# joey156/MECH5845M-WBC-for-Legged-Manipulator

Measured on AMD Instinct MI355X. Metric: wbc_qp_solves_per_sec, higher is better.
Workload: dtype f64

## Files before the change

### mech5845m-wbc-for-legged-manipulator_amd/csrc/wbc_api.hip

```cpp
#include <hip/hip_runtime.h>
#include <stdarg.h>
#include <stdio.h>
#include <string.h>
#include <new>
#include <vector>
#include "wbc_device.h"

using namespace wbc;

static thread_local char g_err[512] = "";
static int fail(int code, const char* fmt, ...) {
  va_list ap;
  va_start(ap, fmt);
  vsnprintf(g_err, sizeof g_err, fmt, ap);
  va_end(ap);
  return code;
}
#define HIP_TRY(expr)                                                                       \
  do {                                                                                      \
    hipError_t e_ = (expr);                                                                 \
    if (e_ != hipSuccess) return fail(WBC_E_HIP, "%s: %s", #expr, hipGetErrorString(e_));   \
  } while (0)

enum TickPath : int { TICK_GENERAL = 0, TICK_SIM3 = 1, TICK_SIM3P = 2, TICK_ORTHP = 3, TICK_BOXP = 4 };
// ... 28 lines not shown
  int packed_min_batch;
  int packed_kernel;
  int posture_par, last_posture_par;
  int packed_box;
  int packed_orth;
  int refine;
  int warm_start;
  int32_t* d_defer;
  unsigned long long* d_dstat;
  int wave_order;
  WaveOrder* d_worder;
  int worder_reset;
  int worder_B;
  uint32_t tick_seq;
  int packed_update, last_update_packed;
  int last_orth;
  int last_qp_path;
  int last_path;
  int max_nj, max_nf;
  int rot;
  unsigned long long* d_prof;
  double *d_pu, *d_pq;
  void* d_roll;
};

static bool is_identity(const double* R) {
  static const double I[9] = {1, 0, 0, 0, 1, 0, 0, 0, 1};
  for (int i = 0; i < 9; ++i)
    if (R[i] != I[i]) return false;
  return true;
// ... 83 lines not shown

extern "C" void wbc_model_destroy(WbcModel* m) { delete m; }

extern "C" void wbc_batch_destroy(WbcBatch* b);
extern "C" int wbc_batch_create(const WbcModel* const* models, int n_models, int max_batch, int device_id, WbcBatch** out) {
  if (!out || n_models < 0 || n_models > WBC_MAX_MODELS || (n_models > 0 && !models) || max_batch < 1)
    return fail(WBC_E_ARG, "wbc_batch_create: bad arguments (n_models %d, max_batch %d)", n_models, max_batch);
  int ndev = 0;
  if (hipGetDeviceCount(&ndev) != hipSuccess || ndev < 1)
    return fail(WBC_E_HIP, "wbc_batch_create: no HIP device visible (this library has no CPU fallback)");
  if (device_id < 0 || device_id >= ndev) return fail(WBC_E_ARG, "wbc_batch_create: device %d of %d", device_id, ndev);
  HIP_TRY(hipSetDevice(device_id));
  WbcBatch* b = new (std::nothrow) WbcBatch;
  if (!b) return fail(WBC_E_ARG, "out of memory");
  memset(b, 0, sizeof *b);
  b->device_id = device_id; b->n_models = n_models; b->max_batch = max_batch; b->presolve = 1; b->presolve_orth = 1; b->packed_update = 1; b->sim3_kernel = 1; b->sing_tol = 1e-7; b->wave_order = 1;
  b->jtj_mfma = -1; b->refine = 1; b->packed_min_batch = WBC_SIM3P_MIN_BATCH; b->warm_start = 0; b->packed_kernel = 1; b->packed_orth = 1; b->packed_box = 1; b->posture_par = 1;
  std::vector<DevModel> dm(n_models);
  for (int i = 0; i < n_models; ++i) {
    if (!models[i]) { delete b; return fail(WBC_E_ARG, "wbc_batch_create: model %d is null", i); }
    b->models[i] = models[i];
    dm[i] = models[i]->dev;
    if (models[i]->blob.njoints > b->max_nj) b->max_nj = models[i]->blob.njoints;
    if (models[i]->blob.nframes > b->max_nf) b->max_nf = models[i]->blob.nframes;
    if (models[i]->dev.rot_mask) b->rot = 1;
  }
#define HIP_TRY_B(expr)                                                                                              \
  do {                                                                                                               \
    hipError_t e_ = (expr);                                                                                          \
    if (e_ != hipSuccess) { wbc_batch_destroy(b); return fail(WBC_E_HIP, "%s: %s", #expr, hipGetErrorString(e_)); }  \
  } while (0)
// ... 100 lines not shown
    if (jp < 0) return;
    if (jp != joint_id && ((M.col_subtree[M.idx_v_of[jp]] >> joint_id) & 1u)) return;
    zero |= 1u << i;
    if (literal) pert |= 1u << qi;
  }
  if (mode == WBC_JOINT_MANI) return;
  P->post_static = 1; P->post_zero = zero; P->post_pert = pert;
  uint32_t dofs = 0;
  for (int k = 0; k < M.nv; ++k) if ((pert >> M.col_q[k]) & 1u) dofs |= 1u << k;
  bool dep = c.con_com != 0 && dofs != 0;
  if (c.con_trunk && (M.frame_support[WBC_FR_TRUNK] & dofs)) dep = true;
  for (int e = 0; e < WBC_NEE; ++e) if (c.con_ee[e] && (M.frame_support[WBC_FR_EE0 + e] & dofs)) dep = true;
  P->post_fk2 = dep ? 1 : 0;
}

static bool build_pk_fk(const DevModel& M, int need_depth, DevPlan* P) {
  for (int i = 0; i < 32; ++i) P->pk_scq[i] = -1;
  for (int L = 0; L < 5; ++L) {
    int cnt = 0;
    for (int i = 0; i < 16; ++i) { memset(&P->pk_fk[L][i], 0, sizeof P->pk_fk[L][i]); P->pk_fk[L][i].joint = -1; }
    for (int j = 2; j < M.njoints; ++j)
      if (M.depth[j] == L + 2 && M.depth[j] <= need_depth) {
        if (cnt < 16) {
          DevPlan::PkJoint& r = P->pk_fk[L][cnt];
          const bool rev = M.jtype[j] >= WBC_JT_RX && M.jtype[j] <= WBC_JT_RZ;
          r.joint = j; r.parent = M.parent[j]; r.a0 = 3 * M.ax0[j]; r.a1 = 3 * M.ax1[j]; r.a2 = 3 * M.ax2[j];
          r.rev = rev ? 1 : 0; r.q_idx = M.idx_q[j]; r.t0 = M.tp[j][0]; r.t1 = M.tp[j][1]; r.t2 = M.tp[j][2]; r.rot = (M.rot_mask >> j) & 1u;
          if (rev && j < 32) P->pk_scq[j] = M.idx_q[j];
        }
        ++cnt;
      }
    if (cnt > 16) return false;
  }
  return true;
}

static bool build_q_tables(const DevModel& M, DevPlan* P, bool need_subtree) {
  if (M.njoints > 22 || M.maxdepth > 7) return false;
  for (int i = 0; i < 32; ++i) { P->q_scq[i] = -1; memset(&P->q_dof[i], 0, sizeof P->q_dof[i]); P->q_dof[i].bl = P->q_dof[i].red = -1; memset(&P->q_jm[i], 0, sizeof P->q_jm[i]); }
  for (int L = 0; L < 6; ++L) {
    int cnt = 0;
    for (int i = 0; i < 16; ++i) { memset(&P->q_fk[L][i], 0, sizeof P->q_fk[L][i]); P->q_fk[L][i].joint = -1; }
    for (int j = 2; j < M.njoints; ++j)
      if (M.depth[j] == L + 2) {
        if (cnt >= 16) return false;
        DevPlan::PkJoint& r = P->q_fk[L][cnt++];
        const bool rev = M.jtype[j] >= WBC_JT_RX && M.jtype[j] <= WBC_JT_RZ;
        r.joint = j; r.parent = M.parent[j]; r.a0 = 3 * M.ax0[j]; r.a1 = 3 * M.ax1[j]; r.a2 = 3 * M.ax2[j];
// ... 232 lines not shown
  b->configured[mi] = true;
  b->plan_host[mi] = DevPlan();
  b->mrows = m; b->prows = p; b->mcart = mcart;
  HIP_TRY(hipMemcpy(b->d_cfgs + mi, cfg, sizeof *cfg, hipMemcpyHostToDevice));
  DevPlan plan;
  build_plan(b->models[mi]->dev, *cfg, p, &plan);
  b->plan_host[mi] = plan;
  HIP_TRY(hipMemcpy(b->d_plans + mi, &plan, sizeof plan, hipMemcpyHostToDevice));
  b->worder_reset = 1;
  return WBC_OK;
}

extern "C" int wbc_task_rows(const WbcBatch* b) { return b ? b->mrows : WBC_E_ARG; }
extern "C" int wbc_constraint_rows(const WbcBatch* b) { return b ? b->prows : WBC_E_ARG; }

extern "C" int wbc_batch_set_option(WbcBatch* b, const char* name, int value) {
  if (!b || !name) return fail(WBC_E_ARG, "wbc_batch_set_option: null");
  if (!strcmp(name, "jtj_mfma")) { b->jtj_mfma = value < 0 ? -1 : (value ? 1 : 0); return WBC_OK; }
  if (!strcmp(name, "presolve")) { b->presolve = value; return WBC_OK; }
  if (!strcmp(name, "presolve_orth")) { b->presolve_orth = value; return WBC_OK; }
  if (!strcmp(name, "orth_qr")) { b->orth_qr = value; return WBC_OK; }
  if (!strcmp(name, "packed_update")) { b->packed_update = value; return WBC_OK; }
  if (!strcmp(name, "presolve_tol_exp")) { double t = 1.0; for (int i = 0; i < value; ++i) t *= 0.1; b->sing_tol = t; return WBC_OK; }
  if (!strcmp(name, "sim3_kernel")) { b->sim3_kernel = value; return WBC_OK; }
  if (!strcmp(name, "packed_kernel")) { b->packed_kernel = value; return WBC_OK; }
  if (!strcmp(name, "wave_order")) { b->wave_order = value < 0 ? 0 : (value > 2 ? 2 : value); return WBC_OK; }
  if (!strcmp(name, "packed_min_batch")) { b->packed_min_batch = value < 1 ? 1 : value; return WBC_OK; }
  if (!strcmp(name, "packed_orth")) { b->packed_orth = value; return WBC_OK; }
  if (!strcmp(name, "packed_box")) { b->packed_box = value; return WBC_OK; }
  if (!strcmp(name, "posture_par")) { b->posture_par = value; return WBC_OK; }
  if (!strcmp(name, "dbg_alias_inputs")) { b->dbg_alias = value; return WBC_OK; }
  if (!strcmp(name, "warm_start")) { b->warm_start = value != 0; return WBC_OK; }
  if (!strcmp(name, "refine")) { b->refine = value > 0; return WBC_OK; }
  if (!strcmp(name, "count_pivoted")) { b->count_pivoted = value != 0; return WBC_OK; }
  if (!strcmp(name, "dbg_force_defer")) { b->force_defer = value != 0; return WBC_OK; }
  if (!strcmp(name, "dbg_stop")) {
#ifdef WBC_ABLATE
    b->dbg_stop = value; return WBC_OK;
#else
    return value == 0 ? WBC_OK : fail(WBC_E_UNSUPPORTED, "dbg_stop needs the ablation build of the library (make -C csrc ablate; WBC_HIP_LIB=.../libwbc_hip_ablate.so)");
#endif
  }
  if (!strcmp(name, "grid")) { if (value < 1) return fail(WBC_E_ARG, "grid must be >= 1"); b->grid = value; return WBC_OK; }
  return fail(WBC_E_ARG, "unknown option %s", name);
}

extern "C" int wbc_batch_get_stat(WbcBatch* b, const char* name, void* stream, int64_t* out) {
  if (!b || !name || !out) return fail(WBC_E_ARG, "wbc_batch_get_stat: null");
  HIP_TRY(hipSetDevice(b->device_id));
  if (!strcmp(name, "last_path")) { *out = b->last_path; return WBC_OK; }
  if (!strcmp(name, "last_qp_path")) { *out = b->last_qp_path; return WBC_OK; }
  if (!strcmp(name, "last_update_packed")) { *out = b->last_update_packed; return WBC_OK; }
  if (!strcmp(name, "last_posture_par")) { *out = b->last_posture_par; return WBC_OK; }
  if (!strcmp(name, "last_orth")) { *out = (b->last_path == TICK_GENERAL || b->last_path == TICK_ORTHP) ? b->last_orth : 0; return WBC_OK; }
  if (!strcmp(name, "deferred_last")) {
    *out = 0;
    if (b->last_path >= TICK_SIM3P) {
      if (!b->d_dstat) return WBC_OK;
      unsigned long long v = 0;
      HIP_TRY(hipStreamSynchronize((hipStream_t)stream));
      HIP_TRY(hipMemcpy(&v, b->d_dstat, sizeof v, hipMemcpyDeviceToHost));
      *out = ((uint32_t)(v >> 32) == b->tick_seq) ? (int64_t)(v & 0xFFFFFFFFull) : 0;
      return WBC_OK;
    }
    if (!b->d_defer || b->last_path == TICK_GENERAL) return WBC_OK;
    int32_t c = 0;
    HIP_TRY(hipStreamSynchronize((hipStream_t)stream));
// ... 153 lines not shown
    }
    if (all_static && !a.in.q_con) { a.post_static = 1; return WBC_OK; }
  }
  if (!b->d_pu) {
    HIP_TRY(hipMalloc((void**)&b->d_pu, sizeof(double) * WBC_V_STRIDE * (size_t)b->max_batch));
    HIP_TRY(hipMalloc((void**)&b->d_pq, sizeof(double) * WBC_Q_STRIDE * (size_t)b->max_batch));
  }
  if (int rc = run_posture(b, B, a.in.q, a.in.model_id, b->d_pu, b->d_pq, stream)) return rc;
  a.in.posture_u = b->d_pu;
  if (literal && !a.in.q_con) a.in.q_con = b->d_pq;
  return WBC_OK;
}

static void fill_args(KernelArgs& a, const WbcBatch* b, int B, double dt) {
  memset(&a, 0, sizeof a);
  a.models = b->d_models; a.cfgs = b->d_cfgs; a.plans = b->d_plans; a.n_models = b->n_models; a.rot = b->rot;
  a.B = B; a.mrows = b->mrows; a.prows = b->prows; a.mcart = b->mcart; a.jtj_mfma = b->jtj_mfma < 0 ? (b->mcart >= WBC_MFMA_AUTO_ROWS) : b->jtj_mfma; a.presolve = b->presolve; a.presolve_orth = b->presolve_orth ? 1 + any_orth_plan(b) : 0; a.orth_qr = b->orth_qr; a.refine = b->refine; a.sing_tol = b->sing_tol; a.dbg_alias = b->dbg_alias; a.dt = dt;
  a.prof = b->d_prof; a.dbg_stop = b->dbg_stop;
  a.fk_nj = b->max_nj; a.fk_nf = b->max_nf;
}

static int launch_rc(int e, const char* what) {
  if (e == WBC_E_UNSUPPORTED) return fail(e, "%s kernel: no variant of it is built for this combination of inputs", what);
  return e ? fail(WBC_E_HIP, "%s kernel launch failed: %s", what, hipGetErrorString((hipError_t)e)) : WBC_OK;
}
static int launch_update_auto(WbcBatch* b, UpdateArgs& u, int B, void* stream) {
  bool packed = b->packed_update != 0;
  for (int i = 0; i < b->n_models && packed; ++i) packed = b->configured[i] && b->plan_host[i].pk_update_ok != 0;
  u.plans = b->d_plans;
  b->last_update_packed = packed;
  return packed ? launch_update_packed(u, stream) : launch_update(u, B, stream);
}
static bool packed_eligible(const WbcBatch* b, const KernelArgs& a) {
  const bool qcon = a.in.q_con || a.in.posture_u;
  bool packed = b->packed_kernel && a.B >= b->packed_min_batch &&
                !b->count_pivoted && !(b->dbg_stop > 0 && b->dbg_stop < 100) && !b->dbg_alias;
  for (int i = 0; i < b->n_models && packed; ++i) packed = qcon ? (b->plan_host[i].packed_ok_pu != 0) : (b->plan_host[i].packed_ok != 0);
  return packed;
}
static bool sim3_eligible(const WbcBatch* b, const KernelArgs& a) {
  if (!b->sim3_kernel || !b->presolve || b->n_models < 1) return false;
  if (b->jtj_mfma > 0) return false;
  if (a.in.com_target || a.in.com_target_vel) return false;
  if (b->prows > WBC_SIM3_MAXP || b->mcart > 12) return false;
// ... 66 lines not shown
        }
      }
      if (b->d_worder && b->worder_reset) {
        HIP_TRY(hipMemsetAsync(b->d_worder, 0, WO_NS * sizeof(WaveOrder), (hipStream_t)stream));
        b->worder_reset = 0;
      }
      a.worder = b->d_worder;
    }
    b->worder_B = a.worder ? a.B : 0;
  }
  return WBC_OK;
}
static int launch_tick_auto(WbcBatch* b, KernelArgs& a, int B, void* stream, const WbcTaskParams* tp = nullptr) {
  const TickPath path = select_tick_path(b, a, tp);
  b->last_path = path;
  if (path == TICK_GENERAL) b->last_orth = a.presolve && a.presolve_orth == 2 && !(a.ws_in || a.ws_out);
  else if (path >= TICK_ORTHP) b->last_orth = path == TICK_ORTHP;
  int rc = prepare_tick(b, a, stream, path);
  if (rc) return rc;
  switch (path) {
    case TICK_GENERAL: return launch_rc(launch_tick(a, MODE_TICK, grid_tick(b, B), stream, tp), "tick");
    case TICK_SIM3P: return launch_rc(launch_tick_sim3p(a, stream, tp), "packed sim3 tick");
    case TICK_ORTHP: return launch_rc(launch_tick_orthp(a, stream, b->plan_host[0].q_ok == 2, tp), "packed orth tick");
    case TICK_BOXP: return launch_rc(launch_tick_boxp(a, stream, tp), "packed box tick");
    case TICK_SIM3: break;
  }
  if ((rc = launch_rc(launch_tick_sim3(a, B, stream), "sim3 tick"))) return rc;
  if ((rc = launch_rc(launch_tick_deferred(a, stream), "deferred tick")))
    (void)hipMemsetAsync(b->d_defer, 0, sizeof(int32_t), (hipStream_t)stream);
  return rc;
// ... 291 lines not shown
```

### mech5845m-wbc-for-legged-manipulator_amd/csrc/wbc_device.h

```cpp
#pragma once
#include <stddef.h>
#include <stdint.h>
#include "../../include/wbc.h"

namespace wbc {

constexpr int NV = WBC_V_STRIDE;
constexpr int NQ = WBC_Q_STRIDE;
constexpr int NL = 32;

struct DevModel {
  int32_t nq, nv, njoints, maxdepth, nframes, pad_[3];
  int32_t parent[NL], depth[NL], jtype[NL], idx_q[NL];
  int32_t ax0[NL], ax1[NL], ax2[NL];
  double tp[NL][3];
  double mass[NL], com[NL][3];
  int32_t col_joint[NL], col_lin[NL], col_ang[NL], col_q[NL];
  uint32_t col_subtree[NL];
  int32_t idx_v_of[NL];
  int32_t frame_joint[WBC_MAX_FRAMES];
  double frame_p[WBC_MAX_FRAMES][3];
  uint32_t frame_support[WBC_MAX_FRAMES];
  double total_mass;
  uint32_t rot_mask, pad1_;
// ... 38 lines not shown
  uint32_t post_pert;
  int32_t mp_ok, mp_n, mp_pad_[2];
  int32_t mp_i[32], mp_qi[32], mp_joint[32];
  int32_t mp_chain[32][8];
  uint32_t mp_prev[32];
  uint32_t mp_all;
  uint32_t mp_prevmode;
  uint32_t flags;
  uint32_t task_ee_mask, con_ee_mask;
  int32_t rowstart[4];
  int32_t legd[12];
  int32_t Fd[WBC_PLAN_NR];
  uint32_t redsup[WBC_MAX_FRAMES];
  int32_t pos[32];
  int32_t lidx[32];
};

enum Mode : int { MODE_TICK = 0, MODE_ASSEMBLE = 1, MODE_FK = 2 };

constexpr int WO_NCLS = 6;
constexpr int WO_SW = 127;
constexpr int WO_CAP = 4 * WO_SW;
constexpr int WO_NS = 256;
struct WaveOrder {
  unsigned long long word[2];
  uint32_t cur;
  uint32_t B;
  uint32_t off[8];
  uint32_t pad_[18];
};
static_assert(sizeof(WaveOrder) == 128, "one slice block per 128-byte line");
inline size_t wave_order_bytes(int max_batch) {
  const int ns = ((max_batch + 3) / 4 + WO_SW - 1) / WO_SW;
  return ns > WO_NS ? 0 : WO_NS * sizeof(WaveOrder) + sizeof(uint32_t) * 2 * WO_NS * WO_NCLS * (size_t)WO_CAP;
}

struct KernelArgs {
  const DevModel* models;
  const WbcConfig* cfgs;
  const DevPlan* plans;
  int32_t B, mrows, prows, mcart;
  int32_t n_models, pad0_;
  int32_t post_static;
  int32_t dbg_alias;
  int32_t dbg_stop;
  int32_t jtj_mfma, presolve;
  int32_t fk_nj, fk_nf;
  int32_t* defer;
  int32_t* pivot_count;
  int32_t* defer_aux;
  int32_t dbg_force_defer;
  int32_t packed_trunk;
  uint32_t tick_seq;
  unsigned long long* defer_stat;
  int32_t presolve_orth;
  int32_t orth_qr;
  int32_t refine;
// ... 48 lines not shown
  const DevModel* models;
  const WbcConfig* cfgs;
  const DevPlan* plans;
  int32_t B, n_models;
  const double* q;
  const int32_t* model_id;
  double *u, *q_after;
  int32_t rot;
};

struct UpdateArgs {
  const DevModel* models;
  const WbcConfig* cfgs;
  const DevPlan* plans;
  int32_t B, n_models;
  int32_t mode, pad_;
  const double *q_cur, *q_next, *imu, *foot_targets;
  const int32_t* model_id;
  double* q_new;
  double *ee_target, *prev_ee_target, *trunk_target, *prev_trunk_target, *ee_prev_rot, *trunk_prev_rot;
  const double *ee_ref_rot, *trunk_ref_euler, *ee_step, *trunk_step;
  double* grip_trace;
  const int32_t *status, *iters;
  int32_t *status_max, *iters_sum;
  int32_t rot;
};

int launch_tick(const KernelArgs& a, int mode, int grid, void* stream, const WbcTaskParams* tp = nullptr);
int launch_tick_sim3(const KernelArgs& a, int grid, void* stream);
int launch_tick_sim3p(const KernelArgs& a, void* stream, const WbcTaskParams* tp = nullptr);
int launch_tick_boxp(const KernelArgs& a, void* stream, const WbcTaskParams* tp = nullptr);
// ... 17 lines not shown
```

### mech5845m-wbc-for-legged-manipulator_amd/csrc/wbc_k_misc.hip

```cpp
#include "wbc_packed.h"

namespace wbc {

template <int NM, bool WARM = false>
__global__ void __launch_bounds__(64, 2) wbc_qp_kernel(const QpArgs A) {
  __shared__ Smem S;
  S.cl[threadIdx.x] = 0.0;
#pragma unroll 1
  for (int b = blockIdx.x; b < A.B; b += gridDim.x) {
    int lane = threadIdx.x, n = A.n, p = A.p, m = A.m;
    asm volatile("" : "+v"(lane), "+s"(n), "+s"(p), "+s"(m));
    const int li = li_clamp(lane);
    double g = 0.0;
    if (m > 0) {
      const double* Ab = A.A + (size_t)b * m * n;
      const double* bb = A.bvec + (size_t)b * m;
      if (A.use_mfma) {
        jtj_mfma(S, lane, m, [&](int r, int c) -> double {
          if (r >= m) return 0.0;
          if (c < n) return Ab[(size_t)r * n + c];
          return (c == NV) ? bb[r] : 0.0;
        });
        g = (lane < n) ? -S.npv[li] : 0.0;
        if (n < NV) {
// ... 722 lines not shown
  const double eet = (A.ee_target && s < 15) ? A.ee_target[b * 15 + s] : 0.0;
  const double ees = (A.ee_target && A.ee_step && s < 15) ? A.ee_step[b * 15 + s] : 0.0;
  double rref[3] = {0.0, 0.0, 0.0};
  if (A.ee_prev_rot && A.ee_ref_rot) {
#pragma unroll
    for (int h = 0; h < 3; ++h) if (16 * h + s < 45) rref[h] = A.ee_ref_rot[b * 45 + 16 * h + s];
  }
  const double tt = (A.trunk_target && s < 3) ? A.trunk_target[b * 3 + s] : 0.0;
  const double tts = (A.trunk_target && A.trunk_step && s < 3) ? A.trunk_step[b * 3 + s] : 0.0;
  const double ter = (A.trunk_prev_rot && A.trunk_ref_euler && s < 3) ? A.trunk_ref_euler[b * 3 + s] : 0.0;
  int st = 0, stm = 0, it = 0, its = 0;
  if (s == 0) {
    if (A.status_max) { st = A.status[b]; stm = A.status_max[b]; }
    if (A.iters_sum) { it = A.iters[b]; its = A.iters_sum[b]; }
  }
  DevPlan::PkJoint fkn = P.pk_fk[0][s];
  const int scq0 = P.pk_scq[(2 + s) & 31], scq1 = P.pk_scq[(18 + s) & 31];
  const int fr = (s < 4) ? WBC_FR_EE0 + s : ((s == 4) ? WBC_FR_TRUNK : WBC_FR_EE0 + 4);
  const int fjoint = M.frame_joint[fr];
  const double f0 = M.frame_p[fr][0], f1 = M.frame_p[fr][1], f2 = M.frame_p[fr][2];
  const int tjoint = M.frame_joint[WBC_FR_TRUNK];
  U.q[s] = c0; U.q[16 + s] = c1;
  if (s < 12) U.ft[s] = ft;
  WSYNC();
  const double* const qv = U.q;
  double* const oMi = U.oMi;
  if (scq0 >= 0) { const SinCos t = sincos_cw(qv[scq0]); U.sc[2 * (2 + s)] = t.s; U.sc[2 * (2 + s) + 1] = t.c; }
  if (scq1 >= 0) { const SinCos t = sincos_cw(qv[scq1]); U.sc[2 * (18 + s)] = t.s; U.sc[2 * (18 + s) + 1] = t.c; }
  if (s == 0) {
    double Rt[9];
    quat_to_R(qv + 3, Rt);
#pragma unroll
    for (int c = 0; c < 3; ++c)
#pragma unroll
      for (int rr = 0; rr < 3; ++rr) oMi[12 + 3 * c + rr] = Rt[3 * rr + c];
    oMi[12 + 9] = qv[0]; oMi[12 + 10] = qv[1]; oMi[12 + 11] = qv[2];
  }
  WSYNC();
#pragma unroll 1
  for (int L = 0; L < 5; ++L) {
    const DevPlan::PkJoint fk = fkn;
    if (L + 1 < 5) fkn = P.pk_fk[L + 1][s];
    const int j = fk.joint;
    if (j >= 0) {
      const bool rev = fk.rev != 0;
      const int a0 = fk.a0, a1 = fk.a1, a2 = fk.a2;
      const double* Pp = oMi + 12 * fk.parent;
      const double sn = rev ? U.sc[2 * j] : 0.0, cs = rev ? U.sc[2 * j + 1] : 1.0;
      const double pris = rev ? 0.0 : qv[fk.q_idx];
      if (ROT && fk.rot) {
        fk_place_rot_lds(oMi + 12 * j, Pp, M.rp[j], a0, a1, a2, sn, cs, pris);
      } else {
        double Av[3], Bv[3], Cv[3], Pv[3];
#pragma unroll
        for (int rr = 0; rr < 3; ++rr) { Av[rr] = Pp[a0 + rr]; Bv[rr] = Pp[a1 + rr]; Cv[rr] = Pp[a2 + rr]; Pv[rr] = Pp[9 + rr]; }
        double* Po = oMi + 12 * j;
#pragma unroll
        for (int rr = 0; rr < 3; ++rr) {
          Po[a0 + rr] = Av[rr];
          Po[a1 + rr] = cs * Bv[rr] + sn * Cv[rr];
          Po[a2 + rr] = cs * Cv[rr] - sn * Bv[rr];
          Po[9 + rr] = Pv[rr] + Av[rr] * (fk.t0 + pris) + Bv[rr] * fk.t1 + Cv[rr] * fk.t2;
        }
      }
    }
    WSYNC();
  }
  if (s < 6) {
    const double* Pj = oMi + 12 * fjoint;
#pragma unroll
    for (int rr = 0; rr < 3; ++rr) U.pf[4 * s + rr] = Pj[9 + rr] + Pj[rr] * f0 + Pj[3 + rr] * f1 + Pj[6 + rr] * f2;
  }
  WSYNC();
  const double* Pt = oMi + 12 * tjoint;
  double WPA[3], BPA[3], base[3];
#pragma unroll
  for (int i = 0; i < 3; ++i) {
    const double t = U.pf[4 * 4 + i];
    WPA[i] = (U.ft[i] + U.ft[3 + i] + U.ft[6 + i] + U.ft[9 + i]) / 4;
    BPA[i] = ((U.pf[i] - t) + (U.pf[4 + i] - t) + (U.pf[8 + i] - t) + (U.pf[12 + i] - t)) / 4;
  }
// ... 86 lines not shown
```

### mech5845m-wbc-for-legged-manipulator_amd/csrc/wbc_k_sim3p.hip

```cpp
#include "wbc_packed.h"

namespace wbc {

#ifdef WBC_ABLATE
#define PSTOP(k, val) do { if (A.dbg_stop == 100 + (k)) { if (valid) { A.out.qdot[(size_t)b * NV + s] = (val); if (s == 0) A.out.status[b] = 0; } return; } } while (0)
#else
#define PSTOP(k, val) do { } while (0)
#endif
#ifndef SIM3P_WAVES
#define SIM3P_WAVES 2
#endif
template <bool WARM, bool TRUNK = false, bool QCON = false, bool ROT = false, bool TP = false>
#ifdef SIM3P_NUM_VGPR
__attribute__((amdgpu_waves_per_eu(SIM3P_NUM_VGPR, SIM3P_NUM_VGPR)))
#endif
__global__ void __launch_bounds__(64, SIM3P_WAVES) wbc_tick_sim3p_kernel(const KernelArgs A, const DevModel* __restrict__ models,
                                                               const WbcConfig* __restrict__ cfgs, const DevPlan* __restrict__ plans,
                                                               const WbcTaskParams* __restrict__ tps) {
#ifdef SIM3P_NUM_VGPR
  extern __shared__ double dyn_lds_[];
  union SUU { SmemP P; Smem G; };
  SUU& SU = *reinterpret_cast<SUU*>(dyn_lds_);
#else
  __shared__ union { SmemP P; Smem G; } SU;
// ... 124 lines not shown
      for (int k = 0; k < 6; ++k) {
        const double2a t0 = lds2(At2 + k * 6), t1 = lds2(At2 + k * 6 + 2), t2 = lds2(At2 + k * 6 + 4);
        I.Cq[s * 6 + k] = fma(at[0], t0.x, fma(at[1], t0.y, fma(at[2], t1.x, fma(at[3], t1.y, fma(at[4], t2.x, at[5] * t2.y)))));
      }
      I.Cq[36 + s] = gs;
    }
    WSYNC();
    __builtin_amdgcn_sched_barrier(0);
  }
  const int nv = M.nv, nq = M.nq, n = P.n_red, nelim = P.nelim, nl = 3 * nelim, p_keep = P.p_keep, p = p_keep + nl;
  const unsigned fl = P.flags;
  const bool c_con_trunk = fl & 2u;
  const int c_task_joint = (fl >> 4) & 7u;
  const bool has_grip = (P.task_ee_mask >> 4) & 1u;
  const DevPlan::PkCol cv = P.pk_var[s], cg = P.pk_leg[s];
  DevPlan::PkJoint fkn = P.pk_fk[0][s];
  const int scq0 = P.pk_scq[(2 + s) & 31], scq1 = P.pk_scq[(18 + s) & 31];
  const int dof0 = cv.dof, dof1 = cg.dof;
  const int c0_joint = cv.joint, c0_lin = cv.lin, c0_ang = cv.ang, c1_joint = cg.joint, c1_lin = cg.lin, c1_ang = cg.ang;
  const int dq0 = cv.dq_idx, dq1 = cg.dq_idx;
  const double dlo0 = cv.d_lo, dhi0 = cv.d_hi, dvm0 = cv.d_vm, dlo1 = cg.d_lo, dhi1 = cg.d_hi, dvm1 = cg.d_vm;
  const double dcoef = cfg.damper_coef, dqi = cfg.damper_qi, dqs = cfg.damper_qs;
  const int gj = M.frame_joint[WBC_FR_EE0 + 4];
  const double gp0 = M.frame_p[WBC_FR_EE0 + 4][0], gp1 = M.frame_p[WBC_FR_EE0 + 4][1], gp2 = M.frame_p[WBC_FR_EE0 + 4][2];
  const unsigned gsup = P.redsup[WBC_FR_EE0 + 4];
  const double ee_w = TPW(ee_w[4]);
  double eW[6], eG[3];
#pragma unroll
  for (int i = 0; i < 6; ++i) eW[i] = TPW(ee_W[4][i]);
#pragma unroll
  for (int i = 0; i < 3; ++i) eG[i] = TPW(ee_gain[4][i]);
// ... 6 lines not shown
  {
    if (scq0 >= 0) { const SinCos t = sincos_cw(qv[scq0]); sc[2 * (2 + s)] = t.s; sc[2 * (2 + s) + 1] = t.c; }
    if (scq1 >= 0) { const SinCos t = sincos_cw(qv[scq1]); sc[2 * (18 + s)] = t.s; sc[2 * (18 + s) + 1] = t.c; }
    if (s == 0) {
      double Rt[9];
      quat_to_R(qv + 3, Rt);
#pragma unroll
      for (int c = 0; c < 3; ++c)
#pragma unroll
        for (int rr = 0; rr < 3; ++rr) oMi[12 + 3 * c + rr] = Rt[3 * rr + c];
      oMi[12 + 9] = qv[0]; oMi[12 + 10] = qv[1]; oMi[12 + 11] = qv[2];
    }
  }
  WSYNC();
  PSTOP(7, oMi[12 + s] + sc[4 + s]);
#pragma unroll 1
  for (int L = 0; L < 5; ++L) {
    const DevPlan::PkJoint fk = fkn;
    if (L + 1 < 5) fkn = P.pk_fk[L + 1][s];
    const int j = fk.joint;
    if (j >= 0) {
      const bool rev = fk.rev != 0;
      const int a0 = fk.a0, a1 = fk.a1, a2 = fk.a2;
      const double* Pp = oMi + 12 * fk.parent;
      const double sn = rev ? sc[2 * j] : 0.0, cs = rev ? sc[2 * j + 1] : 1.0;
      const double pris = rev ? 0.0 : qv[fk.q_idx];
      if (ROT && fk.rot) {
        fk_place_rot_lds(oMi + 12 * j, Pp, M.rp[j], a0, a1, a2, sn, cs, pris);
      } else {
        double Av[3], Bv[3], Cv[3], Pv[3];
#pragma unroll
        for (int rr = 0; rr < 3; ++rr) { Av[rr] = Pp[a0 + rr]; Bv[rr] = Pp[a1 + rr]; Cv[rr] = Pp[a2 + rr]; Pv[rr] = Pp[9 + rr]; }
        double* Po = oMi + 12 * j;
#pragma unroll
        for (int rr = 0; rr < 3; ++rr) {
          Po[a0 + rr] = Av[rr];
          Po[a1 + rr] = cs * Bv[rr] + sn * Cv[rr];
          Po[a2 + rr] = cs * Cv[rr] - sn * Bv[rr];
          Po[9 + rr] = Pv[rr] + Av[rr] * (fk.t0 + pris) + Bv[rr] * fk.t1 + Cv[rr] * fk.t2;
        }
      }
    }
    WSYNC();
  }
  PSTOP(1, oMi[12 * 4 + (s & 7)]);
  double lin0[3] = {0, 0, 0}, ang0[3] = {0, 0, 0}, lin1[3] = {0, 0, 0};
  if (s < n) {
    const double* Pj = oMi + 12 * c0_joint;
    const double pj[3] = {Pj[9], Pj[10], Pj[11]};
    if (c0_ang >= 0) { ang0[0] = Pj[3 * c0_ang]; ang0[1] = Pj[3 * c0_ang + 1]; ang0[2] = Pj[3 * c0_ang + 2]; cross3(pj, ang0, lin0); }
    if (c0_lin >= 0) { lin0[0] = Pj[3 * c0_lin]; lin0[1] = Pj[3 * c0_lin + 1]; lin0[2] = Pj[3 * c0_lin + 2]; }
  }
  if (s < nl) {
    const double* Pj = oMi + 12 * c1_joint;
    const double pj[3] = {Pj[9], Pj[10], Pj[11]};
    if (c1_ang >= 0) { const double a1[3] = {Pj[3 * c1_ang], Pj[3 * c1_ang + 1], Pj[3 * c1_ang + 2]}; cross3(pj, a1, lin1); }
    if (c1_lin >= 0) { lin1[0] = Pj[3 * c1_lin]; lin1[1] = Pj[3 * c1_lin + 1]; lin1[2] = Pj[3 * c1_lin + 2]; }
  }
// ... 95 lines not shown
    for (int k = 0; k < PV; ++k) if (k == s) h[k] += (s < n) ? dpost * dpost : 1.0;
    if (TRUNK && s < 6) {
#pragma unroll
      for (int k = 0; k < 6; k += 2) { const double2a v = lds2(I.Cq + s * 6 + k); h[k] += v.x; h[k + 1] += v.y; }
    }
  }
  PSTOP(2, h[0] + h[5] + h[11] + g);
  if (QCON && A.in.q_con) {
    WSYNC();
    {
      const double* qg = A.in.q_con + (size_t)b * NQ;
      const double c0 = qg[s], c1 = (16 + s < NQ) ? qg[16 + s] : 0.0;
      V.in[s] = c0;
      if (16 + s < 28) V.in[16 + s] = c1;
    }
    fkn = P.pk_fk[0][s];
    WSYNC();
  {
    if (scq0 >= 0) { const SinCos t = sincos_cw(qv[scq0]); sc[2 * (2 + s)] = t.s; sc[2 * (2 + s) + 1] = t.c; }
    if (scq1 >= 0) { const SinCos t = sincos_cw(qv[scq1]); sc[2 * (18 + s)] = t.s; sc[2 * (18 + s) + 1] = t.c; }
    if (s == 0) {
      double Rt[9];
      quat_to_R(qv + 3, Rt);
#pragma unroll
      for (int c = 0; c < 3; ++c)
#pragma unroll
        for (int rr = 0; rr < 3; ++rr) oMi[12 + 3 * c + rr] = Rt[3 * rr + c];
      oMi[12 + 9] = qv[0]; oMi[12 + 10] = qv[1]; oMi[12 + 11] = qv[2];
    }
  }
    WSYNC();
#pragma unroll 1
  for (int L = 0; L < 5; ++L) {
    const DevPlan::PkJoint fk = fkn;
    if (L + 1 < 5) fkn = P.pk_fk[L + 1][s];
    const int j = fk.joint;
    if (j >= 0) {
      const bool rev = fk.rev != 0;
      const int a0 = fk.a0, a1 = fk.a1, a2 = fk.a2;
      const double* Pp = oMi + 12 * fk.parent;
      const double sn = rev ? sc[2 * j] : 0.0, cs = rev ? sc[2 * j + 1] : 1.0;
      const double pris = rev ? 0.0 : qv[fk.q_idx];
      if (ROT && fk.rot) {
        fk_place_rot_lds(oMi + 12 * j, Pp, M.rp[j], a0, a1, a2, sn, cs, pris);
      } else {
        double Av[3], Bv[3], Cv[3], Pv[3];
#pragma unroll
        for (int rr = 0; rr < 3; ++rr) { Av[rr] = Pp[a0 + rr]; Bv[rr] = Pp[a1 + rr]; Cv[rr] = Pp[a2 + rr]; Pv[rr] = Pp[9 + rr]; }
        double* Po = oMi + 12 * j;
#pragma unroll
        for (int rr = 0; rr < 3; ++rr) {
          Po[a0 + rr] = Av[rr];
          Po[a1 + rr] = cs * Bv[rr] + sn * Cv[rr];
          Po[a2 + rr] = cs * Cv[rr] - sn * Bv[rr];
          Po[9 + rr] = Pv[rr] + Av[rr] * (fk.t0 + pris) + Bv[rr] * fk.t1 + Cv[rr] * fk.t2;
        }
      }
    }
    WSYNC();
  }
    lin0[0] = lin0[1] = lin0[2] = 0.0; ang0[0] = ang0[1] = ang0[2] = 0.0; lin1[0] = lin1[1] = lin1[2] = 0.0;
    if (s < n) {
      const double* Pj = oMi + 12 * c0_joint;
      const double pj[3] = {Pj[9], Pj[10], Pj[11]};
      if (c0_ang >= 0) { ang0[0] = Pj[3 * c0_ang]; ang0[1] = Pj[3 * c0_ang + 1]; ang0[2] = Pj[3 * c0_ang + 2]; cross3(pj, ang0, lin0); }
      if (c0_lin >= 0) { lin0[0] = Pj[3 * c0_lin]; lin0[1] = Pj[3 * c0_lin + 1]; lin0[2] = Pj[3 * c0_lin + 2]; }
    }
    if (s < nl) {
      const double* Pj = oMi + 12 * c1_joint;
      const double pj[3] = {Pj[9], Pj[10], Pj[11]};
      if (c1_ang >= 0) { const double a1[3] = {Pj[3 * c1_ang], Pj[3 * c1_ang + 1], Pj[3 * c1_ang + 2]}; cross3(pj, a1, lin1); }
      if (c1_lin >= 0) { lin1[0] = Pj[3 * c1_lin]; lin1[1] = Pj[3 * c1_lin + 1]; lin1[2] = Pj[3 * c1_lin + 2]; }
    }
    {
// ... 842 lines not shown
```

### mech5845m-wbc-for-legged-manipulator_amd/csrc/wbc_packed.h

```cpp
#pragma once
#include "wbc_common.h"

namespace wbc {

constexpr int PLD = 14;
constexpr int PN = 16;
constexpr int PV = 12;
struct __attribute__((aligned(16))) PInst {
  double M1[PV * PLD];
  double M2[PV * PLD];
  double Cq[PN * 6];
  double pad_[8];
};
struct __attribute__((aligned(16))) PVec {
  double in[40];
  double xv[PN], dv[PN], yv[PN], tv[PN];
  double cl[32];
  double pad_[8];
};
static_assert(sizeof(PInst) % 256 == 192, "matrix blocks: 192 B (mod the 256-byte bank row) apart");
static_assert(sizeof(PVec) % 256 == 128, "vector blocks: half a bank row apart (mod 256 B)");
struct __attribute__((aligned(16))) SmemP { PInst I[4]; PVec V[4]; };

__device__ __forceinline__ double rsum16(double v) {
// ... 103 lines not shown
  const uint32_t at = (uint32_t)((old >> (9 * cls)) & 511ull) + (uint32_t)__popc(same & ((1u << r) - 1u));
  if (valid && s == 0 && at < WO_CAP) wo_list(wo, nxt, g, cls)[at] = (uint32_t)b;
  const uint32_t nwaves = (uint32_t)((G - g + ns - 1) / ns);
  if (r == 0 && s == 0 && (uint32_t)(old >> 54) == nwaves - 1u) {
    const unsigned long long fin = old + add;
    uint32_t n = 0u;
#pragma unroll
    for (int c = 0; c < WO_NCLS; ++c) { sl.off[c] = n; n += (uint32_t)((fin >> (9 * c)) & 511ull); }
    const uint32_t expect = 4u * nwaves - ((g == (G - 1) % ns) ? (uint32_t)(4 * G - B) : 0u);
    sl.B = (n == expect) ? (uint32_t)B : 0u;
    sl.cur = nxt;
    sl.word[cur] = 0ull;
  }
}

constexpr int QLEV = 6;
static_assert(offsetof(WbcConfig, joint_w) - offsetof(WbcConfig, ee_W) == 84 * sizeof(double), "ee_W [30] ee_w [5] ee_gain [30] trunk [13] com_W [3] com_gain [3] joint_w");
constexpr int WT_W = 0, WT_w = 30, WT_G = 35, WT_CW = 78, WT_CG = 81;

}
```

Measured before the change: 394.5 million.

## Spread FK joint placement across three lanes per joint in packed kernels

Adds a per-plan table that maps each FK joint at each depth level onto three lanes, one per row component, with precomputed LDS offsets. The packed sim3p and update kernels use this table when the model has no fixed-joint rotations and at most five joints per level, so each lane does a scalar update instead of a three-element loop. The goal is to cut per-lane FK work and index arithmetic in the serial depth sweep. It adds a wave-wide ballot check and a larger DevPlan, and keeps the old sweep as a fallback behind an fk_lanes option.

```diff
diff --git a/mech5845m-wbc-for-legged-manipulator_amd/csrc/wbc_api.hip b/mech5845m-wbc-for-legged-manipulator_amd/csrc/wbc_api.hip
--- a/mech5845m-wbc-for-legged-manipulator_amd/csrc/wbc_api.hip
+++ b/mech5845m-wbc-for-legged-manipulator_amd/csrc/wbc_api.hip
@@ -66,6 +66,7 @@
   int worder_B;
   uint32_t tick_seq;
   int packed_update, last_update_packed;
+  int fk_lanes, last_fk_lanes;
   int last_orth;
   int last_qp_path;
   int last_path;
@@ -179,7 +180,7 @@
   WbcBatch* b = new (std::nothrow) WbcBatch;
   if (!b) return fail(WBC_E_ARG, "out of memory");
   memset(b, 0, sizeof *b);
-  b->device_id = device_id; b->n_models = n_models; b->max_batch = max_batch; b->presolve = 1; b->presolve_orth = 1; b->packed_update = 1; b->sim3_kernel = 1; b->sing_tol = 1e-7; b->wave_order = 1;
+  b->device_id = device_id; b->n_models = n_models; b->max_batch = max_batch; b->presolve = 1; b->presolve_orth = 1; b->packed_update = 1; b->sim3_kernel = 1; b->sing_tol = 1e-7; b->wave_order = 1; b->fk_lanes = 1;
   b->jtj_mfma = -1; b->refine = 1; b->packed_min_batch = WBC_SIM3P_MIN_BATCH; b->warm_start = 0; b->packed_kernel = 1; b->packed_orth = 1; b->packed_box = 1; b->posture_par = 1;
   std::vector<DevModel> dm(n_models);
   for (int i = 0; i < n_models; ++i) {
@@ -310,7 +311,28 @@
   P->post_fk2 = dep ? 1 : 0;
 }
 
+static void build_pk_fk3(const DevModel& M, DevPlan* P) {
+  bool ok = M.rot_mask == 0;
+  for (int L = 0; L < 5; ++L) {
+    if (P->pk_fk[L][5].joint >= 0) ok = false;
+    for (int i = 0; i < 16; ++i) {
+      DevPlan::PkJoint3& r = P->pk_fk3[L][i];
+      memset(&r, 0, sizeof r);
+      r.joint = -1;
+      const DevPlan::PkJoint& f = P->pk_fk[L][i / 3];
+      if (i == 15 || f.joint < 0) continue;
+      const int rr = i % 3, pb = 12 * f.parent;
+      r.joint = f.joint; r.dd = 12 * (f.joint - f.parent);
+      r.ia = pb + f.a0 + rr; r.ib = pb + f.a1 + rr; r.ic = pb + f.a2 + rr; r.ip = pb + 9 + rr;
+      r.q_idx = f.q_idx; r.sc = f.rev ? 2 * f.joint : -1;
+      r.t0 = f.t0; r.t1 = f.t1; r.t2 = f.t2;
+    }
+  }
+  P->pk_fk3_ok = ok ? 1 : 0;
+}
+
 static bool build_pk_fk(const DevModel& M, int need_depth, DevPlan* P) {
+  P->pk_fk3_ok = 0;
   for (int i = 0; i < 32; ++i) P->pk_scq[i] = -1;
   for (int L = 0; L < 5; ++L) {
     int cnt = 0;
@@ -328,6 +350,7 @@
       }
     if (cnt > 16) return false;
   }
+  build_pk_fk3(M, P);
   return true;
 }
 
@@ -590,6 +613,11 @@
 extern "C" int wbc_task_rows(const WbcBatch* b) { return b ? b->mrows : WBC_E_ARG; }
 extern "C" int wbc_constraint_rows(const WbcBatch* b) { return b ? b->prows : WBC_E_ARG; }
 
+static int fk3_plans(const WbcBatch* b) {
+  for (int i = 0; i < b->n_models; ++i) if (!b->configured[i] || !b->plan_host[i].pk_fk3_ok) return 0;
+  return b->n_models > 0;
+}
+
 extern "C" int wbc_batch_set_option(WbcBatch* b, const char* name, int value) {
   if (!b || !name) return fail(WBC_E_ARG, "wbc_batch_set_option: null");
   if (!strcmp(name, "jtj_mfma")) { b->jtj_mfma = value < 0 ? -1 : (value ? 1 : 0); return WBC_OK; }
@@ -601,6 +629,7 @@
   if (!strcmp(name, "sim3_kernel")) { b->sim3_kernel = value; return WBC_OK; }
   if (!strcmp(name, "packed_kernel")) { b->packed_kernel = value; return WBC_OK; }
   if (!strcmp(name, "wave_order")) { b->wave_order = value < 0 ? 0 : (value > 2 ? 2 : value); return WBC_OK; }
+  if (!strcmp(name, "fk_lanes")) { b->fk_lanes = value != 0; return WBC_OK; }
   if (!strcmp(name, "packed_min_batch")) { b->packed_min_batch = value < 1 ? 1 : value; return WBC_OK; }
   if (!strcmp(name, "packed_orth")) { b->packed_orth = value; return WBC_OK; }
   if (!strcmp(name, "packed_box")) { b->packed_box = value; return WBC_OK; }
@@ -627,6 +656,8 @@
   if (!strcmp(name, "last_path")) { *out = b->last_path; return WBC_OK; }
   if (!strcmp(name, "last_qp_path")) { *out = b->last_qp_path; return WBC_OK; }
   if (!strcmp(name, "last_update_packed")) { *out = b->last_update_packed; return WBC_OK; }
+  if (!strcmp(name, "last_fk_lanes")) { *out = b->last_fk_lanes; return WBC_OK; }
+  if (!strcmp(name, "pk_fk3_ok")) { *out = fk3_plans(b); return WBC_OK; }
   if (!strcmp(name, "last_posture_par")) { *out = b->last_posture_par; return WBC_OK; }
   if (!strcmp(name, "last_orth")) { *out = (b->last_path == TICK_GENERAL || b->last_path == TICK_ORTHP) ? b->last_orth : 0; return WBC_OK; }
   if (!strcmp(name, "deferred_last")) {
@@ -810,7 +841,7 @@
 
 static void fill_args(KernelArgs& a, const WbcBatch* b, int B, double dt) {
   memset(&a, 0, sizeof a);
-  a.models = b->d_models; a.cfgs = b->d_cfgs; a.plans = b->d_plans; a.n_models = b->n_models; a.rot = b->rot;
+  a.models = b->d_models; a.cfgs = b->d_cfgs; a.plans = b->d_plans; a.n_models = b->n_models; a.rot = b->rot; a.fk_lanes = b->fk_lanes;
   a.B = B; a.mrows = b->mrows; a.prows = b->prows; a.mcart = b->mcart; a.jtj_mfma = b->jtj_mfma < 0 ? (b->mcart >= WBC_MFMA_AUTO_ROWS) : b->jtj_mfma; a.presolve = b->presolve; a.presolve_orth = b->presolve_orth ? 1 + any_orth_plan(b) : 0; a.orth_qr = b->orth_qr; a.refine = b->refine; a.sing_tol = b->sing_tol; a.dbg_alias = b->dbg_alias; a.dt = dt;
   a.prof = b->d_prof; a.dbg_stop = b->dbg_stop;
   a.fk_nj = b->max_nj; a.fk_nf = b->max_nf;
@@ -823,7 +854,7 @@
 static int launch_update_auto(WbcBatch* b, UpdateArgs& u, int B, void* stream) {
   bool packed = b->packed_update != 0;
   for (int i = 0; i < b->n_models && packed; ++i) packed = b->configured[i] && b->plan_host[i].pk_update_ok != 0;
-  u.plans = b->d_plans;
+  u.plans = b->d_plans; u.fk_lanes = b->fk_lanes;
   b->last_update_packed = packed;
   return packed ? launch_update_packed(u, stream) : launch_update(u, B, stream);
 }
@@ -920,6 +951,7 @@
 static int launch_tick_auto(WbcBatch* b, KernelArgs& a, int B, void* stream, const WbcTaskParams* tp = nullptr) {
   const TickPath path = select_tick_path(b, a, tp);
   b->last_path = path;
+  b->last_fk_lanes = path == TICK_SIM3P && a.fk_lanes && !a.rot && fk3_plans(b);
   if (path == TICK_GENERAL) b->last_orth = a.presolve && a.presolve_orth == 2 && !(a.ws_in || a.ws_out);
   else if (path >= TICK_ORTHP) b->last_orth = path == TICK_ORTHP;
   int rc = prepare_tick(b, a, stream, path);
diff --git a/mech5845m-wbc-for-legged-manipulator_amd/csrc/wbc_device.h b/mech5845m-wbc-for-legged-manipulator_amd/csrc/wbc_device.h
--- a/mech5845m-wbc-for-legged-manipulator_amd/csrc/wbc_device.h
+++ b/mech5845m-wbc-for-legged-manipulator_amd/csrc/wbc_device.h
@@ -76,7 +76,13 @@
   uint32_t redsup[WBC_MAX_FRAMES];
   int32_t pos[32];
   int32_t lidx[32];
-};
+  struct PkJoint3 { int32_t joint, dd, ia, ib, ic, ip, q_idx, sc;
+                    double t0, t1, t2; };
+  PkJoint3 pk_fk3[5][16];
+  int32_t pk_fk3_ok;
+  int32_t pad3_;
+};
+static_assert(sizeof(DevPlan::PkJoint3) == sizeof(DevPlan::PkJoint), "the packed kernels fetch either record through the same registers");
 
 enum Mode : int { MODE_TICK = 0, MODE_ASSEMBLE = 1, MODE_FK = 2 };
 
@@ -102,7 +108,7 @@
   const WbcConfig* cfgs;
   const DevPlan* plans;
   int32_t B, mrows, prows, mcart;
-  int32_t n_models, pad0_;
+  int32_t n_models, fk_lanes;
   int32_t post_static;
   int32_t dbg_alias;
   int32_t dbg_stop;
@@ -181,7 +187,7 @@
   const WbcConfig* cfgs;
   const DevPlan* plans;
   int32_t B, n_models;
-  int32_t mode, pad_;
+  int32_t mode, fk_lanes;
   const double *q_cur, *q_next, *imu, *foot_targets;
   const int32_t* model_id;
   double* q_new;
diff --git a/mech5845m-wbc-for-legged-manipulator_amd/csrc/wbc_k_misc.hip b/mech5845m-wbc-for-legged-manipulator_amd/csrc/wbc_k_misc.hip
--- a/mech5845m-wbc-for-legged-manipulator_amd/csrc/wbc_k_misc.hip
+++ b/mech5845m-wbc-for-legged-manipulator_amd/csrc/wbc_k_misc.hip
@@ -760,7 +760,8 @@
     if (A.status_max) { st = A.status[b]; stm = A.status_max[b]; }
     if (A.iters_sum) { it = A.iters[b]; its = A.iters_sum[b]; }
   }
-  DevPlan::PkJoint fkn = P.pk_fk[0][s];
+  const bool fk3 = !ROT && fk3_wave(A.fk_lanes, P);
+  DevPlan::PkJoint fkn = ROT ? P.pk_fk[0][s] : fk_first(P, s, fk3);
   const int scq0 = P.pk_scq[(2 + s) & 31], scq1 = P.pk_scq[(18 + s) & 31];
   const int fr = (s < 4) ? WBC_FR_EE0 + s : ((s == 4) ? WBC_FR_TRUNK : WBC_FR_EE0 + 4);
   const int fjoint = M.frame_joint[fr];
@@ -783,34 +784,9 @@
     oMi[12 + 9] = qv[0]; oMi[12 + 10] = qv[1]; oMi[12 + 11] = qv[2];
   }
   WSYNC();
-#pragma unroll 1
-  for (int L = 0; L < 5; ++L) {
-    const DevPlan::PkJoint fk = fkn;
-    if (L + 1 < 5) fkn = P.pk_fk[L + 1][s];
-    const int j = fk.joint;
-    if (j >= 0) {
-      const bool rev = fk.rev != 0;
-      const int a0 = fk.a0, a1 = fk.a1, a2 = fk.a2;
-      const double* Pp = oMi + 12 * fk.parent;
-      const double sn = rev ? U.sc[2 * j] : 0.0, cs = rev ? U.sc[2 * j + 1] : 1.0;
-      const double pris = rev ? 0.0 : qv[fk.q_idx];
-      if (ROT && fk.rot) {
-        fk_place_rot_lds(oMi + 12 * j, Pp, M.rp[j], a0, a1, a2, sn, cs, pris);
-      } else {
-        double Av[3], Bv[3], Cv[3], Pv[3];
-#pragma unroll
-        for (int rr = 0; rr < 3; ++rr) { Av[rr] = Pp[a0 + rr]; Bv[rr] = Pp[a1 + rr]; Cv[rr] = Pp[a2 + rr]; Pv[rr] = Pp[9 + rr]; }
-        double* Po = oMi + 12 * j;
-#pragma unroll
-        for (int rr = 0; rr < 3; ++rr) {
-          Po[a0 + rr] = Av[rr];
-          Po[a1 + rr] = cs * Bv[rr] + sn * Cv[rr];
-          Po[a2 + rr] = cs * Cv[rr] - sn * Bv[rr];
-          Po[9 + rr] = Pv[rr] + Av[rr] * (fk.t0 + pris) + Bv[rr] * fk.t1 + Cv[rr] * fk.t2;
-        }
-      }
-    }
-    WSYNC();
+  if (!ROT && fk3) fk_sweep3(oMi, U.sc, qv, &P, s, fk3_of(fkn));
+  else {
+    WBC_FK_SWEEP1(U.sc)
   }
   if (s < 6) {
     const double* Pj = oMi + 12 * fjoint;
diff --git a/mech5845m-wbc-for-legged-manipulator_amd/csrc/wbc_k_sim3p.hip b/mech5845m-wbc-for-legged-manipulator_amd/csrc/wbc_k_sim3p.hip
--- a/mech5845m-wbc-for-legged-manipulator_amd/csrc/wbc_k_sim3p.hip
+++ b/mech5845m-wbc-for-legged-manipulator_amd/csrc/wbc_k_sim3p.hip
@@ -162,7 +162,8 @@
   const int c_task_joint = (fl >> 4) & 7u;
   const bool has_grip = (P.task_ee_mask >> 4) & 1u;
   const DevPlan::PkCol cv = P.pk_var[s], cg = P.pk_leg[s];
-  DevPlan::PkJoint fkn = P.pk_fk[0][s];
+  const bool fk3 = !ROT && fk3_wave(A.fk_lanes, P);
+  DevPlan::PkJoint fkn = ROT ? P.pk_fk[0][s] : fk_first(P, s, fk3);
   const int scq0 = P.pk_scq[(2 + s) & 31], scq1 = P.pk_scq[(18 + s) & 31];
   const int dof0 = cv.dof, dof1 = cg.dof;
   const int c0_joint = cv.joint, c0_lin = cv.lin, c0_ang = cv.ang, c1_joint = cg.joint, c1_lin = cg.lin, c1_ang = cg.ang;
@@ -199,34 +200,9 @@
   }
   WSYNC();
   PSTOP(7, oMi[12 + s] + sc[4 + s]);
-#pragma unroll 1
-  for (int L = 0; L < 5; ++L) {
-    const DevPlan::PkJoint fk = fkn;
-    if (L + 1 < 5) fkn = P.pk_fk[L + 1][s];
-    const int j = fk.joint;
-    if (j >= 0) {
-      const bool rev = fk.rev != 0;
-      const int a0 = fk.a0, a1 = fk.a1, a2 = fk.a2;
-      const double* Pp = oMi + 12 * fk.parent;
-      const double sn = rev ? sc[2 * j] : 0.0, cs = rev ? sc[2 * j + 1] : 1.0;
-      const double pris = rev ? 0.0 : qv[fk.q_idx];
-      if (ROT && fk.rot) {
-        fk_place_rot_lds(oMi + 12 * j, Pp, M.rp[j], a0, a1, a2, sn, cs, pris);
-      } else {
-        double Av[3], Bv[3], Cv[3], Pv[3];
-#pragma unroll
-        for (int rr = 0; rr < 3; ++rr) { Av[rr] = Pp[a0 + rr]; Bv[rr] = Pp[a1 + rr]; Cv[rr] = Pp[a2 + rr]; Pv[rr] = Pp[9 + rr]; }
-        double* Po = oMi + 12 * j;
-#pragma unroll
-        for (int rr = 0; rr < 3; ++rr) {
-          Po[a0 + rr] = Av[rr];
-          Po[a1 + rr] = cs * Bv[rr] + sn * Cv[rr];
-          Po[a2 + rr] = cs * Cv[rr] - sn * Bv[rr];
-          Po[9 + rr] = Pv[rr] + Av[rr] * (fk.t0 + pris) + Bv[rr] * fk.t1 + Cv[rr] * fk.t2;
-        }
-      }
-    }
-    WSYNC();
+  if (!ROT && fk3) fk_sweep3(oMi, sc, qv, &P, s, fk3_of(fkn));
+  else {
+    WBC_FK_SWEEP1(sc)
   }
   PSTOP(1, oMi[12 * 4 + (s & 7)]);
   double lin0[3] = {0, 0, 0}, ang0[3] = {0, 0, 0}, lin1[3] = {0, 0, 0};
@@ -352,7 +328,7 @@
       V.in[s] = c0;
       if (16 + s < 28) V.in[16 + s] = c1;
     }
-    fkn = P.pk_fk[0][s];
+    fkn = ROT ? P.pk_fk[0][s] : fk_first(P, s, fk3);
     WSYNC();
   {
     if (scq0 >= 0) { const SinCos t = sincos_cw(qv[scq0]); sc[2 * (2 + s)] = t.s; sc[2 * (2 + s) + 1] = t.c; }
@@ -368,34 +344,9 @@
     }
   }
     WSYNC();
-#pragma unroll 1
-  for (int L = 0; L < 5; ++L) {
-    const DevPlan::PkJoint fk = fkn;
-    if (L + 1 < 5) fkn = P.pk_fk[L + 1][s];
-    const int j = fk.joint;
-    if (j >= 0) {
-      const bool rev = fk.rev != 0;
-      const int a0 = fk.a0, a1 = fk.a1, a2 = fk.a2;
-      const double* Pp = oMi + 12 * fk.parent;
-      const double sn = rev ? sc[2 * j] : 0.0, cs = rev ? sc[2 * j + 1] : 1.0;
-      const double pris = rev ? 0.0 : qv[fk.q_idx];
-      if (ROT && fk.rot) {
-        fk_place_rot_lds(oMi + 12 * j, Pp, M.rp[j], a0, a1, a2, sn, cs, pris);
-      } else {
-        double Av[3], Bv[3], Cv[3], Pv[3];
-#pragma unroll
-        for (int rr = 0; rr < 3; ++rr) { Av[rr] = Pp[a0 + rr]; Bv[rr] = Pp[a1 + rr]; Cv[rr] = Pp[a2 + rr]; Pv[rr] = Pp[9 + rr]; }
-        double* Po = oMi + 12 * j;
-#pragma unroll
-        for (int rr = 0; rr < 3; ++rr) {
-          Po[a0 + rr] = Av[rr];
-          Po[a1 + rr] = cs * Bv[rr] + sn * Cv[rr];
-          Po[a2 + rr] = cs * Cv[rr] - sn * Bv[rr];
-          Po[9 + rr] = Pv[rr] + Av[rr] * (fk.t0 + pris) + Bv[rr] * fk.t1 + Cv[rr] * fk.t2;
-        }
-      }
-    }
-    WSYNC();
+  if (!ROT && fk3) fk_sweep3(oMi, sc, qv, &P, s, fk3_of(fkn));
+  else {
+    WBC_FK_SWEEP1(sc)
   }
     lin0[0] = lin0[1] = lin0[2] = 0.0; ang0[0] = ang0[1] = ang0[2] = 0.0; lin1[0] = lin1[1] = lin1[2] = 0.0;
     if (s < n) {
diff --git a/mech5845m-wbc-for-legged-manipulator_amd/csrc/wbc_packed.h b/mech5845m-wbc-for-legged-manipulator_amd/csrc/wbc_packed.h
--- a/mech5845m-wbc-for-legged-manipulator_amd/csrc/wbc_packed.h
+++ b/mech5845m-wbc-for-legged-manipulator_amd/csrc/wbc_packed.h
@@ -141,6 +141,67 @@
   }
 }
 
+#define WBC_FK_SWEEP1(sc) \
+_Pragma("unroll 1")                                                                                                                \
+  for (int L = 0; L < 5; ++L) {                                                                                                    \
+    const DevPlan::PkJoint fk = fkn;                                                                                               \
+    if (L + 1 < 5) fkn = P.pk_fk[L + 1][s];                                                                                        \
+    const int j = fk.joint;                                                                                                        \
+    if (j >= 0) {                                                                                                                  \
+      const bool rev = fk.rev != 0;                                                                                                \
+      const int a0 = fk.a0, a1 = fk.a1, a2 = fk.a2;                                                                                \
+      const double* Pp = oMi + 12 * fk.parent;                                                                                     \
+      const double sn = rev ? sc[2 * j] : 0.0, cs = rev ? sc[2 * j + 1] : 1.0;                                                     \
+      const double pris = rev ? 0.0 : qv[fk.q_idx];                                                                                \
+      if (ROT && fk.rot) {                                                                                                         \
+        fk_place_rot_lds(oMi + 12 * j, Pp, M.rp[j], a0, a1, a2, sn, cs, pris);                                                     \
+      } else {                                                                                                                     \
+        double Av[3], Bv[3], Cv[3], Pv[3];                                                                                         \
+_Pragma("unroll")                                                                                                                  \
+        for (int rr = 0; rr < 3; ++rr) { Av[rr] = Pp[a0 + rr]; Bv[rr] = Pp[a1 + rr]; Cv[rr] = Pp[a2 + rr]; Pv[rr] = Pp[9 + rr]; }  \
+        double* Po = oMi + 12 * j;                                                                                                 \
+_Pragma("unroll")                                                                                                                  \
+        for (int rr = 0; rr < 3; ++rr) {                                                                                           \
+          Po[a0 + rr] = Av[rr];                                                                                                    \
+          Po[a1 + rr] = cs * Bv[rr] + sn * Cv[rr];                                                                                 \
+          Po[a2 + rr] = cs * Cv[rr] - sn * Bv[rr];                                                                                 \
+          Po[9 + rr] = Pv[rr] + Av[rr] * (fk.t0 + pris) + Bv[rr] * fk.t1 + Cv[rr] * fk.t2;                                         \
+        }                                                                                                                          \
+      }                                                                                                                            \
+    }                                                                                                                              \
+    WSYNC();                                                                                                                       \
+  }
+__device__ __forceinline__ void fk_sweep3(double* const oMi, const double* const sc, const double* const qv, const DevPlan* const P, const int s,
+                                          DevPlan::PkJoint3 fkn) {
+#pragma unroll 1
+  for (int L = 0; L < 5; ++L) {
+    const DevPlan::PkJoint3 fk = fkn;
+    if (L + 1 < 5) fkn = P->pk_fk3[L + 1][s];
+    if (fk.joint >= 0) {
+      const bool rev = fk.sc >= 0;
+      const double sn = rev ? sc[fk.sc] : 0.0, cs = rev ? sc[fk.sc + 1] : 1.0;
+      const double pris = rev ? 0.0 : qv[fk.q_idx];
+      const double Av = oMi[fk.ia], Bv = oMi[fk.ib], Cv = oMi[fk.ic], Pv = oMi[fk.ip];
+      double* const Po = oMi + fk.dd;
+      Po[fk.ia] = Av;
+      Po[fk.ib] = fma(cs, Bv, sn * Cv);
+      Po[fk.ic] = fma(cs, Cv, -(sn * Bv));
+      Po[fk.ip] = fma(Cv, fk.t2, fma(Bv, fk.t1, fma(Av, fk.t0 + pris, Pv)));
+    }
+    WSYNC();
+  }
+}
+__device__ __forceinline__ bool fk3_wave(const int fk_lanes, const DevPlan& P) {
+  return __ballot(!(fk_lanes && P.pk_fk3_ok)) == 0ull;
+}
+__device__ __forceinline__ DevPlan::PkJoint fk_first(const DevPlan& P, const int s, const bool fk3) {
+  const void* const src = fk3 ? static_cast<const void*>(&P.pk_fk3[0][s]) : static_cast<const void*>(&P.pk_fk[0][s]);
+  DevPlan::PkJoint f;
+  __builtin_memcpy(&f, src, sizeof f);
+  return f;
+}
+__device__ __forceinline__ DevPlan::PkJoint3 fk3_of(const DevPlan::PkJoint& f) { return __builtin_bit_cast(DevPlan::PkJoint3, f); }
+
 constexpr int QLEV = 6;
 static_assert(offsetof(WbcConfig, joint_w) - offsetof(WbcConfig, ee_W) == 84 * sizeof(double), "ee_W [30] ee_w [5] ee_gain [30] trunk [13] com_W [3] com_gain [3] joint_w");
 constexpr int WT_W = 0, WT_w = 30, WT_G = 35, WT_CW = 78, WT_CG = 81;
```

New measurement: 410.1 million (median of 6 runs). 1.04x the previous value.
